# featureform/embeddinghub

Hardware: NVIDIA H100
Metric: k-NN queries/s (higher is better)
Workload: dtype f32

## Files before the change

embeddinghub_b200/csrc/search.cu:

```cuda
#include <cstdio>

#include "kernels.h"

namespace ehb {

cudaError_t launch_search(const WalkPlan& p, const GraphView& g, const float* queries, uint32_t nq, uint32_t k,
                          uint32_t ef, const ResultSink& sink, uint32_t* out_counts, uint32_t* stats, cudaStream_t s) {
  if (nq == 0) return cudaSuccess;
  if (p.bf16 && (!g.vecs16 || !sink.keys)) return cudaErrorInvalidValue;
  return with_dpad(g.dpad, [&](auto d) {
    constexpr uint32_t D = decltype(d)::value;
    return p.bf16 ? SearchShape<D, __nv_bfloat16>::launch(p, g, queries, nq, k, ef, sink, out_counts, stats, s)
                  : SearchShape<D, float>::launch(p, g, queries, nq, k, ef, sink, out_counts, stats, s);
  });
}

cudaError_t beam_warps(const WalkPlan& p, const GraphView& g, int sms, uint64_t nq, uint32_t* warps) {
  return with_dpad(g.dpad, [&](auto d) {
    constexpr uint32_t D = decltype(d)::value;
    return p.bf16 ? BeamShape<D, __nv_bfloat16>::warps(p, sms, nq, warps) : BeamShape<D, float>::warps(p, sms, nq, warps);
  });
}

cudaError_t resident_warps(const void* kern, uint32_t smem, int sms, uint32_t* out) {
  cudaError_t e = cudaFuncSetAttribute(kern, cudaFuncAttributeMaxDynamicSharedMemorySize, (int)smem);
  int per_sm = 0;
  if (e == cudaSuccess) e = cudaOccupancyMaxActiveBlocksPerMultiprocessor(&per_sm, kern, 32, smem);
  if (e != cudaSuccess) return e;
  if (per_sm < 1) return cudaErrorInvalidConfiguration;
  *out = (uint32_t)per_sm * (uint32_t)sms;
  return cudaSuccess;
}

cudaError_t launch_search_beam(const WalkPlan& p, const GraphView& g, const float* queries, uint32_t nq, uint32_t k,
                               uint32_t ef, const ResultSink& sink, uint32_t* out_counts, uint32_t* stats,
                               uint32_t* vtab, uint32_t warps, cudaStream_t s) {
  if (nq == 0) return cudaSuccess;
  if (p.bf16 && (!g.vecs16 || !sink.keys)) return cudaErrorInvalidValue;
  return with_dpad(g.dpad, [&](auto d) {
    constexpr uint32_t D = decltype(d)::value;
    return p.bf16 ? BeamShape<D, __nv_bfloat16>::launch(p, g, queries, nq, k, ef, sink, out_counts, stats, vtab, warps, s)
                  : BeamShape<D, float>::launch(p, g, queries, nq, k, ef, sink, out_counts, stats, vtab, warps, s);
  });
}

void walk_kernel_name(const WalkPlan& p, char* out, size_t out_bytes) {
  if (p.form == WalkForm::team)
    std::snprintf(out, out_bytes, "hnsw_search_team_kernel<NQ=%d,KPL=%d,T=%u,U=%u>", p.nq, p.kpl, p.T, p.U);
  else if (p.form == WalkForm::beam)
    std::snprintf(out, out_bytes, "hnsw_search_beam_kernel<LPV=%d,NQ=%d%s%s>", p.lpv, p.nq,
                  p.hasdel ? ",HASDEL=1" : "", p.bf16 ? ",ROW=bf16" : "");
  else
    std::snprintf(out, out_bytes, "%s<LPV=%d,NQ=%d,KPL=%d%s%s>",
                  p.form == WalkForm::dense  ? "hnsw_search_dense_kernel"
                  : p.form == WalkForm::wide ? "hnsw_search_wide_kernel"
                                             : "hnsw_search_kernel",
                  p.lpv, p.nq, p.kpl, p.hasdel ? ",HASDEL=1" : "", p.bf16 ? ",ROW=bf16" : "");
}

__global__ void pad_rows_kernel(const float* __restrict__ in, float* __restrict__ out, uint64_t n, uint32_t dim,
                                uint32_t dpad, int normalize) {
  uint64_t row = (uint64_t)blockIdx.x * (blockDim.x >> 5) + (threadIdx.x >> 5);
  uint32_t lane = threadIdx.x & 31;
  if (row >= n) return;
  const float* src = in + row * dim;
  float* dst = out + row * dpad;
  float inv = 1.0f;
  if (normalize) {
    float acc = 0.f;
    if (lane == 0) {
      for (uint32_t i = 0; i < dim; ++i) acc = fmaf(src[i], src[i], acc);
      inv = 1.0f / (sqrtf(acc) + 1e-30f);
    }
    inv = __shfl_sync(0xffffffffu, inv, 0);
  }
  for (uint32_t i = lane; i < dpad; i += 32) dst[i] = i < dim ? (normalize ? src[i] * inv : src[i]) : 0.f;
}

cudaError_t launch_pad_rows(const float* in, float* out, uint64_t n, uint32_t dim, uint32_t dpad, bool normalize,
                            cudaStream_t s) {
  if (n == 0) return cudaSuccess;
  uint32_t wpb = 8;
  pad_rows_kernel<<<(unsigned)((n + wpb - 1) / wpb), 32 * wpb, 0, s>>>(in, out, n, dim, dpad, normalize ? 1 : 0);
  return cudaGetLastError();
}

cudaError_t launch_normalize(const float* in, uint32_t in_stride, float* out, uint32_t out_stride, uint64_t n,
                             uint32_t dim, cudaStream_t s) {
  (void)in_stride;
  return launch_pad_rows(in, out, n, dim, out_stride, true, s);
}

__global__ void to_i8_rows_kernel(const float* __restrict__ in, uint32_t dpad, int8_t* __restrict__ codes,
                                  float4* __restrict__ terms, uint64_t n) {
  const uint64_t row = (uint64_t)blockIdx.x * (blockDim.x >> 5) + (threadIdx.x >> 5);
  const uint32_t lane = threadIdx.x & 31;
  if (row >= n) return;
  const float* src = in + row * dpad;
  float mx = 0.f;
  bool finite = true;
  for (uint32_t i = 4 * lane; i < dpad; i += 128) {
    const float4 v = *(const float4*)(src + i);
    finite = finite && isfinite(v.x) && isfinite(v.y) && isfinite(v.z) && isfinite(v.w);
    mx = fmaxf(mx, fmaxf(fmaxf(fabsf(v.x), fabsf(v.y)), fmaxf(fabsf(v.z), fabsf(v.w))));
  }
  finite = __all_sync(0xffffffffu, finite);
  mx = __uint_as_float(__reduce_max_sync(0xffffffffu, __float_as_uint(mx)));
  const float s = (float)((double)mx / 127.0);
  const bool bad = !finite || (s != 0.f && s < 0x1p-126f);
  const double sd = s;
  double rinf = 0.0, r2 = 0.0, x2 = 0.0;
  for (uint32_t i = 4 * lane; i < dpad; i += 128) {
    const float4 v = *(const float4*)(src + i);
    const float xv[4] = {v.x, v.y, v.z, v.w};
    uint32_t packed = 0;
#pragma unroll
    for (int j = 0; j < 4; ++j) {
      const double x = xv[j];
      const double c = bad || s == 0.f ? 0.0 : fmin(fmax(rint(x / sd), -127.0), 127.0);
      const double r = x - sd * c;
      rinf = fmax(rinf, fabs(r));
      r2 = fma(r, r, r2);
      x2 = fma(x, x, x2);
      packed |= (uint32_t)(uint8_t)(int8_t)c << (8 * j);
    }
    *(uint32_t*)(codes + row * dpad + i) = packed;
  }
#pragma unroll
  for (int o = 16; o > 0; o >>= 1) {
    rinf = fmax(rinf, __shfl_xor_sync(0xffffffffu, rinf, o));
    r2 += __shfl_xor_sync(0xffffffffu, r2, o);
    x2 += __shfl_xor_sync(0xffffffffu, x2, o);
  }
  if (lane == 0) {
    const double up = 1.0 + 0x1p-30;
    terms[row] = bad ? make_float4(NAN, NAN, NAN, NAN)
                     : make_float4(s, __double2float_ru(rinf), __double2float_ru(sqrt(r2) * up),
                                   __double2float_ru(sqrt(x2) * up));
  }
}

cudaError_t launch_to_i8(const float* in, uint32_t dpad, int8_t* codes, float4* terms, uint64_t n, cudaStream_t s) {
  if (n == 0) return cudaSuccess;
  to_i8_rows_kernel<<<(unsigned)((n + 7) / 8), 256, 0, s>>>(in, dpad, codes, terms, n);
  return cudaGetLastError();
}

__global__ void sum_stats_kernel(const uint32_t* __restrict__ stats, uint32_t nq, unsigned long long* out) {
  unsigned long long a[kStatWords] = {};
  for (uint32_t i = blockIdx.x * blockDim.x + threadIdx.x; i < nq; i += gridDim.x * blockDim.x) {
    const uint4 s = ((const uint4*)stats)[2 * i], t = ((const uint4*)stats)[2 * i + 1];
    a[0] += s.x, a[1] += s.y, a[2] += s.z, a[3] += s.w ? 1 : 0, a[4] += t.x, a[5] += t.y;
  }
#pragma unroll
  for (int j = 0; j < 6; ++j) {
    for (int o = 16; o > 0; o >>= 1) a[j] += __shfl_xor_sync(0xffffffffu, a[j], o);
    if ((threadIdx.x & 31) == 0) atomicAdd(&out[j], a[j]);
  }
}

cudaError_t launch_sum_stats(const uint32_t* stats, uint32_t nq, unsigned long long* out, cudaStream_t s) {
  cudaError_t e = cudaMemsetAsync(out, 0, kStatWords * sizeof(unsigned long long), s);
  if (e != cudaSuccess) return e;
  if (nq) sum_stats_kernel<<<64, 256, 0, s>>>(stats, nq, out);
  return cudaGetLastError();
}

}
```

embeddinghub_b200/csrc/search_impl.cuh:

```cuda
#pragma once
#include "kernels.h"

namespace ehb {

template <int LPV, int NQ, int KPL, bool HASDEL, int UDIV, class RowT>
__device__ __forceinline__ void search_body(const GraphView& g, const WalkCfg& cfg, const float* __restrict__ queries,
                                            uint32_t nq, uint32_t k, uint32_t ef, const ResultSink& sink,
                                            uint32_t* __restrict__ out_counts, uint32_t* __restrict__ stats,
                                            uint32_t warp_smem) {
  extern __shared__ __align__(128) unsigned char smem[];
  const uint32_t w = threadIdx.x >> 5;
  const uint32_t q = blockIdx.x * (blockDim.x >> 5) + w;
  if (q >= nq) return;
  constexpr bool kKeys = !std::is_same<RowT, float>::value;
  constexpr bool kScreen = !kKeys && screen_shape(LPV, NQ);
  WarpCtx c;
  ctx_init(c, smem + (size_t)w * warp_smem, cfg, g.dpad, (uint32_t)sizeof(RowT));
  float4 qr[NQ];
  if constexpr (wide_shape(LPV, NQ))
    load_query_smem<NQ, RowT>(c, queries + (size_t)q * g.dim, g.dim);
  else
    load_query_regs<LPV, NQ, RowT>(qr, queries + (size_t)q * g.dim, g.dim, c.lane);
  WalkCounters wc = {0, 0, 0, 0};
  UList<KPL> ul;
  ul_clear<KPL>(ul, ef, c.lane);
  if (g.n != 0) {
    uint32_t cur = g.entry;
    if (c.lane == 0) c.cand_id[0] = cur;
    __syncwarp();
    eval_candidates<LPV, NQ, UDIV, RowT, kScreen>(c, walk_rows<RowT>(g), qr, 1, g.metric);
    float curdist = c.cand_dist[0];
    __syncwarp();
    wc.evals = 1;
    greedy_descent<LPV, NQ, UDIV, RowT, kScreen>(c, g, qr, cur, curdist, g.max_level, 0, wc);
    beam_search<LPV, NQ, KPL, true, HASDEL, UDIV, RowT, kScreen>(c, g, qr, ul, cur, curdist, 0, ef, kInvalid, wc);
  }
  uint64_t rk[KPL];
#pragma unroll
  for (int s = 0; s < KPL; ++s) rk[s] = kMaxKey;
  uint32_t found = 0;
  for (uint32_t i = 0; i < k; ++i) {
    uint64_t key = ul_extract_min<KPL>(ul, c.lane);
    if (key == kMaxKey) break;
#pragma unroll
    for (int s = 0; s < KPL; ++s)
      if ((i >> 5) == (uint32_t)s && (i & 31u) == c.lane) rk[s] = key;
    found++;
  }
  if constexpr (kKeys) {
#pragma unroll
    for (int s = 0; s < KPL; ++s) {
      const uint32_t idx = (uint32_t)s * 32u + c.lane;
      if ((uint32_t)s * 32u < k && idx < k) sink.keys[(size_t)q * k + idx] = rk[s];
    }
  } else {
#pragma unroll
    for (int s = 0; s < KPL; ++s) {
      const uint32_t idx = (uint32_t)s * 32u + c.lane;
      if ((uint32_t)s * 32u < k && idx < k) {
        const bool ok = rk[s] != kMaxKey;
        const uint64_t lab = ok ? g.labels[key_id(rk[s])] : 0xFFFFFFFFFFFFFFFFull;
        const float dist = ok ? key_dist(rk[s]) : INFINITY;
        sink_store(sink, (size_t)q * k + idx, lab, dist);
      }
    }
    sink_query_done(sink, q, nq, c.lane);
  }
  if (c.lane == 0) {
    if (out_counts) out_counts[q] = found;
    if (stats) {
      ((uint4*)stats)[2 * q] = make_uint4(wc.hops_upper, wc.hops_base, wc.evals, wc.overflow);
      ((uint4*)stats)[2 * q + 1] = make_uint4(wc.screened, wc.survivors, 0u, 0u);
    }
  }
}

template <class RowT>
constexpr int kWalkMinBlocks = std::is_same<RowT, float>::value ? 0 : 1;
template <int LPV, int NQ, int KPL, bool HASDEL, class RowT>
__global__ void __launch_bounds__(128, (kWalkMinBlocks<RowT>))
    hnsw_search_kernel(GraphView g, WalkCfg cfg, const float* __restrict__ queries, uint32_t nq, uint32_t k, uint32_t ef,
                       const __grid_constant__ ResultSink sink, uint32_t* __restrict__ out_counts,
                       uint32_t* __restrict__ stats, uint32_t warp_smem) {
  search_body<LPV, NQ, KPL, HASDEL, 1, RowT>(g, cfg, queries, nq, k, ef, sink, out_counts, stats, warp_smem);
}

template <int NQ, int KPL>
constexpr int kScreenWalkRegs = NQ <= 6 && KPL <= 8 ? 200 : 255;
template <int LPV, int NQ, int KPL, bool HASDEL>
__global__ void __maxnreg__((kScreenWalkRegs<NQ, KPL>))
    hnsw_search_screen_kernel(GraphView g, WalkCfg cfg, const float* __restrict__ queries, uint32_t nq, uint32_t k,
                              uint32_t ef, const __grid_constant__ ResultSink sink, uint32_t* __restrict__ out_counts,
                              uint32_t* __restrict__ stats, uint32_t warp_smem) {
  search_body<LPV, NQ, KPL, HASDEL, 1, float>(g, cfg, queries, nq, k, ef, sink, out_counts, stats, warp_smem);
}

template <int LPV, int NQ, int KPL, class RowT>
__global__ void __launch_bounds__(128, 5) hnsw_search_dense_kernel(GraphView g, WalkCfg cfg,
                                                                   const float* __restrict__ queries, uint32_t nq,
                                                                   uint32_t k, uint32_t ef,
                                                                   const __grid_constant__ ResultSink sink,
                                                                   uint32_t* __restrict__ out_counts,
                                                                   uint32_t* __restrict__ stats, uint32_t warp_smem) {
  search_body<LPV, NQ, KPL, false, 2, RowT>(g, cfg, queries, nq, k, ef, sink, out_counts, stats, warp_smem);
}

template <int NQ, int KPL, bool HASDEL, class RowT>
__global__ void __launch_bounds__(128, (kWalkMinBlocks<RowT>))
    hnsw_search_wide_kernel(GraphView g, WalkCfg cfg, const float* __restrict__ queries, uint32_t nq, uint32_t k,
                            uint32_t ef, const __grid_constant__ ResultSink sink, uint32_t* __restrict__ out_counts,
                            uint32_t* __restrict__ stats, uint32_t warp_smem) {
  search_body<32, NQ, KPL, HASDEL, 1, RowT>(g, cfg, queries, nq, k, ef, sink, out_counts, stats, warp_smem);
}

using WalkKernel = void (*)(GraphView, WalkCfg, const float*, uint32_t, uint32_t, uint32_t, const ResultSink,
                           uint32_t*, uint32_t*, uint32_t);
template <int LPV, int NQ, int KPL, class RowT>
WalkKernel walk_kernel(const WalkPlan& p) {
  constexpr bool kBf16 = !std::is_same<RowT, float>::value;
  if constexpr (wide_shape(LPV, NQ)) {
    if (p.form != WalkForm::wide) return nullptr;
    return p.hasdel ? hnsw_search_wide_kernel<NQ, KPL, true, RowT> : hnsw_search_wide_kernel<NQ, KPL, false, RowT>;
  } else {
    if (p.form == WalkForm::wide) return nullptr;
    if (p.form == WalkForm::dense) {
      if constexpr (dense_form(kBf16, LPV, NQ, KPL, false))
        if (!p.hasdel) return hnsw_search_dense_kernel<LPV, NQ, KPL, RowT>;
      return nullptr;
    }
    if constexpr (std::is_same<RowT, float>::value && screen_shape(LPV, NQ))
      return p.hasdel ? hnsw_search_screen_kernel<LPV, NQ, KPL, true> : hnsw_search_screen_kernel<LPV, NQ, KPL, false>;
    else
      return p.hasdel ? hnsw_search_kernel<LPV, NQ, KPL, true, RowT> : hnsw_search_kernel<LPV, NQ, KPL, false, RowT>;
  }
}

template <int LPV, int NQ, int KPL, class RowT>
cudaError_t launch_search_t(const WalkPlan& p, const GraphView& g, const float* queries, uint32_t nq, uint32_t k,
                            uint32_t ef, const ResultSink& sink, uint32_t* out_counts, uint32_t* stats,
                            cudaStream_t s) {
  const uint32_t wpb = p.wpb;
  uint32_t wsm = warp_smem_bytes(p.cfg, g.dpad, (uint32_t)sizeof(RowT));
  size_t smem = (size_t)wsm * wpb;
  dim3 grid((nq + wpb - 1) / wpb), block(32 * wpb);
  const WalkKernel kern = walk_kernel<LPV, NQ, KPL, RowT>(p);
  if (!kern) return cudaErrorInvalidValue;
  cudaError_t e = cudaFuncSetAttribute(kern, cudaFuncAttributeMaxDynamicSharedMemorySize, (int)smem);
  if (e != cudaSuccess) return e;
  kern<<<grid, block, smem, s>>>(g, p.cfg, queries, nq, k, ef, sink, out_counts, stats, wsm);
  return cudaGetLastError();
}

template <uint32_t DPAD, class RowT>
cudaError_t SearchShape<DPAD, RowT>::launch(const WalkPlan& p, const GraphView& g, const float* queries, uint32_t nq,
                                            uint32_t k, uint32_t ef, const ResultSink& sink, uint32_t* out_counts,
                                            uint32_t* stats, cudaStream_t s) {
  constexpr int LPV = row_lpv(DPAD * sizeof(RowT)), NQ = row_nq(DPAD, DPAD * sizeof(RowT));
  if (p.lpv != LPV || p.nq != NQ || p.form == WalkForm::team) return cudaErrorInvalidValue;
  switch (p.kpl) {
    case 2: return launch_search_t<LPV, NQ, 2, RowT>(p, g, queries, nq, k, ef, sink, out_counts, stats, s);
    case 4: return launch_search_t<LPV, NQ, 4, RowT>(p, g, queries, nq, k, ef, sink, out_counts, stats, s);
    case 8: return launch_search_t<LPV, NQ, 8, RowT>(p, g, queries, nq, k, ef, sink, out_counts, stats, s);
    case 16: return launch_search_t<LPV, NQ, 16, RowT>(p, g, queries, nq, k, ef, sink, out_counts, stats, s);
    default: return cudaErrorInvalidValue;
  }
}

}
```

embeddinghub_b200/csrc/walk.cuh:

```cuda
#pragma once
#include <cuda_bf16.h>

#include <type_traits>

#include "common.cuh"

namespace ehb {

struct GraphView {
  const float* vecs;
  const uint32_t* links0;
  const uint32_t* up_off;
  const uint32_t* links_up;
  const uint64_t* labels;
  const uint8_t* deleted;
  uint32_t n, dim, dpad, M, M0, entry;
  int32_t max_level;
  int32_t metric;
  const __nv_bfloat16* vecs16;
  const int8_t* codes8;
  const float4* terms8;
};

struct WalkCfg {
// ... 180 lines not shown
  constexpr int V = LaneChunks<RowT, NQ>::V;
  uint32_t sub = lane % LPV;
#pragma unroll
  for (int t = 0; t < NQ; ++t) {
    uint32_t e = (sub + LPV * (t / V)) * 4u * V + 4u * (t % V);
    float4 v;
    v.x = e + 0 < dim ? src[e + 0] : 0.f;
    v.y = e + 1 < dim ? src[e + 1] : 0.f;
    v.z = e + 2 < dim ? src[e + 2] : 0.f;
    v.w = e + 3 < dim ? src[e + 3] : 0.f;
    qr[t] = v;
  }
}
template <int LPV, int NQ, class RowT, class C = LaneChunks<RowT, NQ>>
__device__ __forceinline__ void load_vec_regs(typename C::T (&r)[C::N], const RowT* __restrict__ row,
                                              uint32_t lane) {
  const typename C::T* p = (const typename C::T*)row + (lane % LPV);
#pragma unroll
  for (int t = 0; t < C::N; ++t) r[t] = p[LPV * t];
}

template <int NQ>
__device__ __forceinline__ float partial_dist(const float4 (&v)[NQ], const float4 (&qr)[NQ], int metric) {
  float a0 = 0.f, a1 = 0.f, a2 = 0.f, a3 = 0.f;
  if (metric == 0) {
#pragma unroll
    for (int t = 0; t < NQ; ++t) {
      float dx = qr[t].x - v[t].x, dy = qr[t].y - v[t].y, dz = qr[t].z - v[t].z, dw = qr[t].w - v[t].w;
      a0 = fmaf(dx, dx, a0);
      a1 = fmaf(dy, dy, a1);
      a2 = fmaf(dz, dz, a2);
      a3 = fmaf(dw, dw, a3);
    }
  } else {
#pragma unroll
    for (int t = 0; t < NQ; ++t) {
      a0 = fmaf(qr[t].x, v[t].x, a0);
      a1 = fmaf(qr[t].y, v[t].y, a1);
      a2 = fmaf(qr[t].z, v[t].z, a2);
      a3 = fmaf(qr[t].w, v[t].w, a3);
    }
  }
  return (a0 + a1) + (a2 + a3);
}
template <int LPV>
__device__ __forceinline__ float group_reduce(float acc) {
#pragma unroll
  for (int o = LPV / 2; o > 0; o >>= 1) acc += __shfl_xor_sync(0xffffffffu, acc, o);
  return acc;
}

template <int NQ, class RowT, class C = LaneChunks<RowT, NQ>>
__device__ __forceinline__ float chunk_dist(const typename C::T (&v)[C::N], const float4 (&qr)[NQ], int metric) {
  float4 x[NQ];
#pragma unroll
  for (int j = 0; j < C::N; ++j) widen(v[j], x + j * C::V);
  return partial_dist<NQ>(x, qr, metric);
}
template <class RowT>
__device__ __forceinline__ const RowT* walk_rows(const GraphView& g) {
  if constexpr (std::is_same<RowT, float>::value)
    return g.vecs;
  else
    return g.vecs16;
}

__host__ __device__ constexpr int eval_u(int N, int UDIV) {
  return ((N <= 2 ? 8 : (N <= 4 ? 4 : 2)) / UDIV) > 0 ? (N <= 2 ? 8 : (N <= 4 ? 4 : 2)) / UDIV : 1;
}
template <int NQ, int U = eval_u(NQ, 1), class RowT = float>
__device__ __forceinline__ void eval_direct(WarpCtx& c, const RowT* __restrict__ rows, const float4 (&qr)[NQ],
                                            uint32_t m, int metric) {
  using C = LaneChunks<RowT, NQ>;
  const uint32_t sub = c.lane & 7u, grp = c.lane >> 3;
  __syncwarp();
#pragma unroll 1
  for (uint32_t j0 = 0; j0 < m; j0 += 4 * U) {
    typename C::T v[U][C::N];
#pragma unroll
    for (int u = 0; u < U; ++u) {
      if (j0 + 4u * u < m) {
        uint32_t j = min(j0 + 4u * u + grp, m - 1u);
        const typename C::T* p = (const typename C::T*)(rows + (size_t)c.cand_id[j] * c.dpad) + sub;
#pragma unroll
        for (int t = 0; t < C::N; ++t) v[u][t] = ld_chunk(p + 8 * t);
      }
    }
#pragma unroll
    for (int u = 0; u < U; ++u) {
      if (j0 + 4u * u < m) {
        uint32_t j = j0 + 4u * u + grp;
        float acc = group_reduce<8>(chunk_dist<NQ, RowT>(v[u], qr, metric));
        if (sub == 0 && j < m) c.cand_dist[j] = metric == 0 ? acc : 1.0f - acc;
      }
    }
  }
  __syncwarp();
}

template <class RowT>
__device__ __forceinline__ void issue_rows(WarpCtx& c, const RowT* __restrict__ vecs, uint32_t r, uint32_t m,
                                           uint32_t G, uint32_t vbytes) {
  uint32_t buf = r % c.NG;
  uint32_t first = r * G;
  uint32_t cnt = min(G, m - first);
  if (c.lane == 0) mbar_arrive_expect_tx(&c.mbar[buf], cnt * vbytes);
  __syncwarp();
  if (c.lane < cnt) {
    uint32_t id = c.cand_id[first + c.lane];
    bulk_g2s((RowT*)c.stage + (size_t)(buf * G + c.lane) * c.dpad, vecs + (size_t)id * c.dpad, vbytes, &c.mbar[buf]);
  }
}
template <class RowT>
__device__ __forceinline__ void issue_group(WarpCtx& c, const RowT* __restrict__ vecs, uint32_t r, uint32_t m) {
  issue_rows(c, vecs, r, m, c.G, c.vbytes);
}
template <int NQ, class RowT>
__device__ __forceinline__ void eval_staged(WarpCtx& c, const RowT* __restrict__ vecs, const float4 (&qr)[NQ],
                                            uint32_t m, int metric) {
  const uint32_t rounds = (m + c.G - 1) / c.G;
  const uint32_t pre = min(rounds, c.NG);
  for (uint32_t r = 0; r < pre; ++r) issue_group(c, vecs, r, m);
#pragma unroll 1
  for (uint32_t r = 0; r < rounds; ++r) {
    uint32_t buf = r % c.NG;
    mbar_wait(&c.mbar[buf], (c.phases >> buf) & 1u);
    c.phases ^= (1u << buf);
    uint32_t first = r * c.G;
    uint32_t cnt = min(c.G, m - first);
#pragma unroll 1
    for (uint32_t v0 = 0; v0 < cnt; v0 += 4) {
      float acc[4];
#pragma unroll
      for (int i = 0; i < 4; ++i) {
        uint32_t v = min(v0 + (uint32_t)i, cnt - 1u);
        typename LaneChunks<RowT, NQ>::T x[LaneChunks<RowT, NQ>::N];
        load_vec_regs<32, NQ>(x, (const RowT*)c.stage + (size_t)(buf * c.G + v) * c.dpad, c.lane);
        acc[i] = chunk_dist<NQ, RowT>(x, qr, metric);
      }
#pragma unroll
      for (int o = 16; o > 0; o >>= 1) {
#pragma unroll
        for (int i = 0; i < 4; ++i) acc[i] += __shfl_xor_sync(0xffffffffu, acc[i], o);
      }
      if (c.lane < 4 && v0 + c.lane < cnt) {
        float a = c.lane == 0 ? acc[0] : (c.lane == 1 ? acc[1] : (c.lane == 2 ? acc[2] : acc[3]));
        c.cand_dist[first + v0 + c.lane] = metric == 0 ? a : 1.0f - a;
      }
    }
    __syncwarp();
    if (r + c.NG < rounds) {
      fence_proxy_async();
      issue_group(c, vecs, r + c.NG, m);
    }
  }
  __syncwarp();
}

template <int NQ>
__device__ __forceinline__ void eval_regs(WarpCtx& c, const float* __restrict__ vecs, const float4 (&qr)[NQ],
                                          uint32_t m, int metric) {
  constexpr int SB = NQ <= 24 ? 24 / NQ : 1;
#pragma unroll 1
  for (uint32_t v0 = 0; v0 < m; v0 += SB) {
    float4 x[SB][NQ];
#pragma unroll
    for (int i = 0; i < SB; ++i) {
      const uint32_t v = min(v0 + (uint32_t)i, m - 1u);
      const float4* p = (const float4*)(vecs + (size_t)c.cand_id[v] * c.dpad) + c.lane;
#pragma unroll
      for (int t = 0; t < NQ; ++t) x[i][t] = ld_nc_f4(p + 32 * t);
    }
    float acc[SB];
#pragma unroll
    for (int i = 0; i < SB; ++i) acc[i] = chunk_dist<NQ, float>(x[i], qr, metric);
#pragma unroll
    for (int o = 16; o > 0; o >>= 1) {
#pragma unroll
      for (int i = 0; i < SB; ++i) acc[i] += __shfl_xor_sync(0xffffffffu, acc[i], o);
    }
    if (c.lane < (uint32_t)SB && v0 + c.lane < m) {
      float a = acc[0];
#pragma unroll
      for (int i = 1; i < SB; ++i)
        if (c.lane == (uint32_t)i) a = acc[i];
      c.cand_dist[v0 + c.lane] = metric == 0 ? a : 1.0f - a;
    }
  }
  __syncwarp();
}

template <int NQ, class RowT>
__device__ __forceinline__ void load_query_smem(WarpCtx& c, const float* __restrict__ src, uint32_t dim) {
  constexpr int V = LaneChunks<RowT, NQ>::V;
  float4* qs = (float4*)c.stage + c.lane;
  __syncwarp();
#pragma unroll 4
  for (int t = 0; t < NQ; ++t) {
    const uint32_t e = (c.lane + 32u * (t / V)) * 4u * V + 4u * (t % V);
    float4 v;
    v.x = e + 0 < dim ? src[e + 0] : 0.f;
    v.y = e + 1 < dim ? src[e + 1] : 0.f;
    v.z = e + 2 < dim ? src[e + 2] : 0.f;
    v.w = e + 3 < dim ? src[e + 3] : 0.f;
    qs[32 * t] = v;
  }
  __syncwarp();
}
constexpr int kWideRows = 4;
template <int NQ, class RowT>
__device__ __forceinline__ void eval_wide(WarpCtx& c, const RowT* __restrict__ vecs, uint32_t m, int metric) {
  using C = LaneChunks<RowT, NQ>;
  constexpr int V = C::V, SB = kWideRows, NS = 8 / V;
  static_assert(C::N % NS == 0, "the d-slices tile the row");
  const float4* qs = (const float4*)c.stage + c.lane;
#pragma unroll 1
  for (uint32_t v0 = 0; v0 < m; v0 += SB) {
    const typename C::T* p[SB];
#pragma unroll
    for (int i = 0; i < SB; ++i)
      p[i] = (const typename C::T*)(vecs + (size_t)c.cand_id[min(v0 + (uint32_t)i, m - 1u)] * c.dpad) + c.lane;
    float a[SB][4];
#pragma unroll
    for (int i = 0; i < SB; ++i) a[i][0] = a[i][1] = a[i][2] = a[i][3] = 0.f;
#pragma unroll 1
    for (int j0 = 0; j0 < C::N; j0 += NS) {
      typename C::T x[SB][NS];
#pragma unroll
      for (int i = 0; i < SB; ++i)
#pragma unroll
        for (int j = 0; j < NS; ++j) x[i][j] = ld_chunk(p[i] + 32 * (j0 + j));
#pragma unroll
      for (int j = 0; j < NS; ++j) {
        float4 q[V];
#pragma unroll
        for (int v = 0; v < V; ++v) q[v] = qs[32 * ((j0 + j) * V + v)];
#pragma unroll
        for (int i = 0; i < SB; ++i) {
          float4 r[V];
          widen(x[i][j], r);
#pragma unroll
          for (int v = 0; v < V; ++v) {
            if (metric == 0) {
              const float dx = q[v].x - r[v].x, dy = q[v].y - r[v].y, dz = q[v].z - r[v].z, dw = q[v].w - r[v].w;
              a[i][0] = fmaf(dx, dx, a[i][0]);
              a[i][1] = fmaf(dy, dy, a[i][1]);
              a[i][2] = fmaf(dz, dz, a[i][2]);
              a[i][3] = fmaf(dw, dw, a[i][3]);
            } else {
              a[i][0] = fmaf(q[v].x, r[v].x, a[i][0]);
              a[i][1] = fmaf(q[v].y, r[v].y, a[i][1]);
              a[i][2] = fmaf(q[v].z, r[v].z, a[i][2]);
              a[i][3] = fmaf(q[v].w, r[v].w, a[i][3]);
            }
          }
        }
      }
    }
    float acc[SB];
#pragma unroll
    for (int i = 0; i < SB; ++i) acc[i] = (a[i][0] + a[i][1]) + (a[i][2] + a[i][3]);
#pragma unroll
    for (int o = 16; o > 0; o >>= 1) {
#pragma unroll
      for (int i = 0; i < SB; ++i) acc[i] += __shfl_xor_sync(0xffffffffu, acc[i], o);
    }
    if (c.lane < (uint32_t)SB && v0 + c.lane < m) {
      float d = acc[0];
#pragma unroll
      for (int i = 1; i < SB; ++i)
        if (c.lane == (uint32_t)i) d = acc[i];
      c.cand_dist[v0 + c.lane] = metric == 0 ? d : 1.0f - d;
    }
  }
  __syncwarp();
}

template <int LPV, int NQ, int UDIV = 1, class RowT = float, bool SCREEN = false>
__device__ __forceinline__ void eval_candidates(WarpCtx& c, const RowT* __restrict__ vecs, const float4 (&qr)[NQ],
                                                uint32_t m, int metric) {
  if constexpr (wide_shape(LPV, NQ)) {
    eval_wide<NQ, RowT>(c, vecs, m, metric);
    return;
  }
  if (LPV == 8) {
    eval_direct<NQ, eval_u(LaneChunks<RowT, NQ>::N, UDIV)>(c, vecs, qr, m, metric);
  } else {
    if constexpr (SCREEN) {
      if (!c.staged) {
        eval_regs<NQ>(c, vecs, qr, m, metric);
        return;
      }
    }
    eval_staged<NQ>(c, vecs, qr, m, metric);
  }
}

constexpr int kQMax = 8191;
struct ScreenQuery {
  float l1, l2, a, en, sq;
};
__device__ __forceinline__ ScreenQuery* screen_query(const WarpCtx& c) { return (ScreenQuery*)(c.mbar + 8); }
template <int NQ>
__device__ __forceinline__ uint32_t screen_regs(WarpCtx& c, const GraphView& g, const uint32_t (&qh)[NQ],
                                                const uint32_t (&ql)[NQ], uint32_t m, uint32_t worst_hi,
                                                uint32_t& unsure) {
  constexpr int RB = 96 / NQ;
  const bool in = c.lane < m;
  const uint32_t id = in ? c.cand_id[c.lane] : kInvalid;
  float4 tm = make_float4(0.f, 0.f, 0.f, 0.f);
  if (in) tm = ld_nc_f4(g.terms8 + id);
  int K = 0;
#pragma unroll 1
  for (uint32_t v0 = 0; v0 < m; v0 += RB) {
    uint32_t x[RB][NQ];
#pragma unroll
    for (int i = 0; i < RB; ++i) {
      const uint32_t* p = (const uint32_t*)(g.codes8 + (size_t)c.cand_id[min(v0 + (uint32_t)i, m - 1u)] * c.dpad) +
                          c.lane;
#pragma unroll
      for (int t = 0; t < NQ; ++t) x[i][t] = ld_nc_u32(p + 32 * t);
    }
#pragma unroll
    for (int i = 0; i < RB; ++i) {
      int h = 0, l = 0;
#pragma unroll
      for (int t = 0; t < NQ; ++t) {
        h = __dp4a((int)x[i][t], (int)qh[t], h);
        l = __dp4a((int)x[i][t], (int)ql[t], l);
      }
      const int kv = __reduce_add_sync(0xffffffffu, 128 * h + l);
      if (c.lane == v0 + (uint32_t)i) K = kv;
    }
  }
  float L = 0.f;
  if (in) {
    const ScreenQuery sq = *screen_query(c);
    const float e = (float)c.dpad * 0x1p-24f;
    const float gam = __fdiv_ru(e, 1.0f - e);
    const float se = __fmul_ru(__fmul_ru(tm.x, __int2float_ru(K)), sq.sq);
    float mg = __fmul_ru(__fmul_ru(gam, sq.l2), tm.w);
    mg = __fadd_ru(mg, fminf(__fmul_ru(sq.l1, tm.y), __fmul_ru(sq.l2, tm.z)));
    mg = __fadd_ru(mg, __fmaf_ru(sq.en, __fadd_ru(tm.w, tm.z), sq.a));
    L = __fsub_rd(__fsub_rd(1.0f, se), mg);
  }
  const bool keep = in && !(isfinite(L) && f2ord(L) >= worst_hi);
  const uint32_t mask = __ballot_sync(0xffffffffu, keep);
  const uint32_t pos = __popc(mask & lanemask_lt());
  __syncwarp();
  if (keep) c.cand_id[pos] = id;
  if (unsure) unsure = __reduce_or_sync(0xffffffffu, (keep && ((unsure >> c.lane) & 1u)) ? (1u << pos) : 0u);
  __syncwarp();
  return __popc(mask);
}

template <int KPL>
struct UList {
  uint32_t hi[KPL];
  uint32_t id[KPL];
};
template <int KPL>
__device__ __forceinline__ void ul_clear(UList<KPL>& u, uint32_t ef, uint32_t lane) {
#pragma unroll
  for (int s = 0; s < KPL; ++s) {
    u.hi[s] = ((uint32_t)s * 32u + lane) < ef ? 0xFFFFFFFFu : 0u;
    u.id[s] = kInvalid;
  }
}
template <int KPL>
__device__ __forceinline__ uint32_t ul_worst(const UList<KPL>& u) {
  uint32_t m = u.hi[0];
#pragma unroll
  for (int s = 1; s < KPL; ++s) m = max(m, u.hi[s]);
  return __reduce_max_sync(0xffffffffu, m);
}
template <int KPL>
__device__ __forceinline__ void ul_insert(UList<KPL>& u, uint32_t hi, uint32_t id, uint32_t ef, uint32_t& cnt,
                                          uint32_t& worst_hi, uint32_t lane) {
  bool done = false;
  if (cnt < ef) {
#pragma unroll
    for (int s = 0; s < KPL; ++s) {
      if (!done) {
        uint32_t b = __ballot_sync(0xffffffffu, u.id[s] == kInvalid && u.hi[s] == 0xFFFFFFFFu);
        if (b) {
          if ((int)lane == __ffs(b) - 1) u.hi[s] = hi, u.id[s] = id;
          done = true;
        }
      }
    }
    cnt++;
    if (cnt == ef) worst_hi = ul_worst<KPL>(u);
  } else {
#pragma unroll
    for (int s = 0; s < KPL; ++s) {
      if (!done) {
        uint32_t b = __ballot_sync(0xffffffffu, u.hi[s] == worst_hi && u.id[s] != kInvalid);
        if (b) {
          if ((int)lane == __ffs(b) - 1) u.hi[s] = hi, u.id[s] = id;
          done = true;
        }
      }
    }
    worst_hi = ul_worst<KPL>(u);
  }
}
template <int KPL>
__device__ __forceinline__ uint32_t ul_min_unexpanded(UList<KPL>& u, bool mark, uint32_t lane) {
  uint32_t m = 0xFFFFFFFFu;
#pragma unroll
  for (int s = 0; s < KPL; ++s)
    if (!(u.id[s] & kExpandedFlag)) m = min(m, u.hi[s]);
  m = __reduce_min_sync(0xffffffffu, m);
  uint32_t node = kInvalid;
  bool done = false;
#pragma unroll
  for (int s = 0; s < KPL; ++s) {
    if (!done) {
      uint32_t b = __ballot_sync(0xffffffffu, !(u.id[s] & kExpandedFlag) && u.hi[s] == m);
      if (b) {
        int l = __ffs(b) - 1;
        node = __shfl_sync(0xffffffffu, u.id[s], l);
        if (mark && (int)lane == l) u.id[s] |= kExpandedFlag;
        done = true;
      }
    }
  }
  return node;
}
template <int KPL>
__device__ __forceinline__ uint32_t ul_min_unexpanded_hi(const UList<KPL>& u) {
  uint32_t m = 0xFFFFFFFFu;
#pragma unroll
  for (int s = 0; s < KPL; ++s)
    if (!(u.id[s] & kExpandedFlag)) m = min(m, u.hi[s]);
  return __reduce_min_sync(0xffffffffu, m);
}
template <int KPL>
__device__ __forceinline__ bool ul_contains(const UList<KPL>& u, uint32_t id) {
  bool hit = false;
#pragma unroll
  for (int s = 0; s < KPL; ++s) hit |= u.id[s] != kInvalid && (u.id[s] & kIdMask) == id;
  return __any_sync(0xffffffffu, hit);
}
template <int KPL>
__device__ __forceinline__ uint64_t ul_extract_min(UList<KPL>& u, uint32_t lane) {
  uint32_t m = 0xFFFFFFFFu;
#pragma unroll
  for (int s = 0; s < KPL; ++s)
    if (u.id[s] != kInvalid) m = min(m, u.hi[s]);
  m = __reduce_min_sync(0xffffffffu, m);
  uint64_t out = kMaxKey;
  bool done = false;
#pragma unroll
  for (int s = 0; s < KPL; ++s) {
    if (!done) {
      uint32_t b = __ballot_sync(0xffffffffu, u.id[s] != kInvalid && u.hi[s] == m);
      if (b) {
        int l = __ffs(b) - 1;
        uint32_t id = __shfl_sync(0xffffffffu, u.id[s], l);
        out = ((uint64_t)m << 32) | (id & kIdMask);
        if ((int)lane == l) u.id[s] = kInvalid, u.hi[s] = 0xFFFFFFFFu;
        done = true;
      }
    }
  }
  return out;
}
template <int KPL>
__device__ __forceinline__ void ul_extract_all(WarpCtx& c, UList<KPL>& u) {
  c.cnt = 0;
  for (;;) {
    uint64_t key = ul_extract_min<KPL>(u, c.lane);
    if (key == kMaxKey) break;
    if (c.lane == 0) c.keys[c.cnt] = key;
    c.cnt++;
  }
  __syncwarp();
}

struct SList {
  uint32_t* hi;
  uint32_t* id;
  uint32_t C;
  uint32_t whi, wrow;
  uint32_t uhi, urow;
};
__device__ __forceinline__ void sl_init(SList& u, const WarpCtx& c) {
  u.hi = (uint32_t*)c.keys;
  u.id = u.hi + c.lcap;
  u.C = c.lcap / 32u;
}
__device__ __forceinline__ void sl_scan(SList& u, uint32_t col, bool worst, uint32_t lane) {
  __syncwarp();
  const uint32_t* hc = u.hi + col * u.C;
  const uint32_t* ic = u.id + col * u.C;
  uint32_t wh = 0, wr = kInvalid, uh = 0xFFFFFFFFu, ur = kInvalid;
  for (uint32_t r = lane; r < u.C; r += 32) {
    const uint32_t h = hc[r], d = ic[r];
    if (d != kInvalid && (wr == kInvalid || h > wh)) wh = h, wr = r;
    if (!(d & kExpandedFlag) && (ur == kInvalid || h < uh)) uh = h, ur = r;
  }
  const uint32_t um = __reduce_min_sync(0xffffffffu, ur != kInvalid ? uh : 0xFFFFFFFFu);
  const uint32_t ub = __ballot_sync(0xffffffffu, ur != kInvalid && uh == um);
  const uint32_t urow = ub ? __shfl_sync(0xffffffffu, ur, __ffs(ub) - 1) : kInvalid;
  if (lane == col) u.uhi = um, u.urow = urow;
  if (worst) {
    const uint32_t wm = __reduce_max_sync(0xffffffffu, wr != kInvalid ? wh : 0u);
    const uint32_t wb = __ballot_sync(0xffffffffu, wr != kInvalid && wh == wm);
    const uint32_t wrow = wb ? __shfl_sync(0xffffffffu, wr, __ffs(wb) - 1) : kInvalid;
    if (lane == col) u.whi = wm, u.wrow = wrow;
  }
}
__device__ __forceinline__ void ul_clear(SList& u, uint32_t ef, uint32_t lane) {
  (void)ef;
  __syncwarp();
  for (uint32_t i = lane; i < 32u * u.C; i += 32) u.hi[i] = 0, u.id[i] = kInvalid;
  u.whi = 0, u.wrow = kInvalid, u.uhi = 0xFFFFFFFFu, u.urow = kInvalid;
  __syncwarp();
}
__device__ __forceinline__ void ul_insert(SList& u, uint32_t hi, uint32_t id, uint32_t ef, uint32_t& cnt,
                                          uint32_t& worst_hi, uint32_t lane) {
  if (cnt < ef) {
    const uint32_t col = cnt & 31u, row = cnt >> 5;
    if (lane == col) {
      u.hi[col * u.C + row] = hi, u.id[col * u.C + row] = id;
      if (u.wrow == kInvalid || hi > u.whi) u.whi = hi, u.wrow = row;
      if (u.urow == kInvalid || hi < u.uhi) u.uhi = hi, u.urow = row;
    }
    __syncwarp();
    cnt++;
    if (cnt == ef) worst_hi = __reduce_max_sync(0xffffffffu, u.wrow != kInvalid ? u.whi : 0u);
  } else {
    const uint32_t b = __ballot_sync(0xffffffffu, u.wrow != kInvalid && u.whi == worst_hi);
    const uint32_t col = __ffs(b) - 1;
    const uint32_t row = __shfl_sync(0xffffffffu, u.wrow, col);
    if (lane == col) u.hi[col * u.C + row] = hi, u.id[col * u.C + row] = id;
    sl_scan(u, col, true, lane);
    worst_hi = __reduce_max_sync(0xffffffffu, u.wrow != kInvalid ? u.whi : 0u);
  }
}
__device__ __forceinline__ uint64_t sl_take_min(SList& u, bool mark, uint32_t lane) {
  const uint32_t m = __reduce_min_sync(0xffffffffu, u.urow != kInvalid ? u.uhi : 0xFFFFFFFFu);
  const uint32_t b = __ballot_sync(0xffffffffu, u.urow != kInvalid && u.uhi == m);
  if (!b) return kMaxKey;
  const uint32_t col = __ffs(b) - 1;
  const uint32_t at = col * u.C + __shfl_sync(0xffffffffu, u.urow, col);
  const uint32_t node = u.id[at];
  if (mark) {
    __syncwarp();
    if (lane == col) u.id[at] = node | kExpandedFlag;
    sl_scan(u, col, false, lane);
  }
  return ((uint64_t)m << 32) | node;
}
__device__ __forceinline__ uint32_t ul_min_unexpanded(SList& u, bool mark, uint32_t lane) {
  const uint64_t key = sl_take_min(u, mark, lane);
  return key == kMaxKey ? kInvalid : (uint32_t)key;
}
__device__ __forceinline__ uint32_t ul_min_unexpanded_hi(const SList& u) {
  return __reduce_min_sync(0xffffffffu, u.urow != kInvalid ? u.uhi : 0xFFFFFFFFu);
}
__device__ __forceinline__ bool ul_contains(const SList& u, uint32_t id) {
  bool hit = false;
  for (uint32_t i = (uint32_t)threadIdx.x & 31u; i < 32u * u.C; i += 32) hit |= u.id[i] != kInvalid && (u.id[i] & kIdMask) == id;
  return __any_sync(0xffffffffu, hit);
}
__device__ __forceinline__ void sl_begin_extract(SList& u, uint32_t lane) {
  __syncwarp();
  for (uint32_t i = lane; i < 32u * u.C; i += 32)
    if (u.id[i] != kInvalid) u.id[i] &= kIdMask;
  for (uint32_t col = 0; col < 32; ++col) sl_scan(u, col, false, lane);
}

__device__ __forceinline__ uint32_t list_insert(WarpCtx& c, uint64_t key, uint32_t limit) {
  const uint32_t id = key_id(key);
  uint32_t pos = 0;
  uint32_t dup = 0;
  for (uint32_t base = 0; base < c.cnt; base += 32) {
    uint32_t i = base + c.lane;
    uint64_t k = i < c.cnt ? c.keys[i] : kMaxKey;
    pos += __popc(__ballot_sync(0xffffffffu, k < key));
    dup |= __ballot_sync(0xffffffffu, i < c.cnt && key_id(k) == id);
  }
  if (dup || pos >= limit) return kInvalid;
  const uint32_t newcnt = min(c.cnt + 1u, limit);
  for (int base = (int)((newcnt - 1u) & ~31u); base >= (int)(pos & ~31u); base -= 32) {
    uint32_t i = (uint32_t)base + c.lane;
    bool in = i >= pos && i < newcnt;
    uint64_t v = key;
    if (in && i > pos) v = c.keys[i - 1];
    __syncwarp();
    if (in) c.keys[i] = v;
  }
  __syncwarp();
  c.cnt = newcnt;
  return pos;
}

struct WalkCounters {
  uint32_t hops_upper, hops_base, evals, overflow, screened, survivors;
};

__device__ __forceinline__ uint32_t load_row(const GraphView& g, uint32_t node, int level, uint32_t lane) {
  const uint32_t* row;
  uint32_t width;
  if (level == 0) {
    row = g.links0 + (size_t)node * g.M0;
    width = g.M0;
  } else {
    row = g.links_up + (size_t)(g.up_off[node] + (uint32_t)(level - 1)) * g.M;
    width = g.M;
  }
  uint32_t v = row[min(lane, width - 1u)];
  return lane < width ? v : kInvalid;
}

template <int LPV, int NQ, int UDIV = 1, class RowT = float, bool SCREEN = false>
__device__ __forceinline__ void greedy_descent(WarpCtx& c, const GraphView& g, const float4 (&qr)[NQ], uint32_t& cur,
                                               float& curdist, int from_level, int to_level_excl,
                                               WalkCounters& wc) {
  for (int level = from_level; level > to_level_excl; --level) {
    bool changed = true;
    while (changed) {
      changed = false;
      __syncwarp();
      uint32_t nb = load_row(g, cur, level, c.lane);
      uint32_t mask = __ballot_sync(0xffffffffu, nb != kInvalid);
      uint32_t m = __popc(mask);
      wc.hops_upper++;
      if (!m) break;
      if (nb != kInvalid) c.cand_id[__popc(mask & lanemask_lt())] = nb;
      __syncwarp();
      wc.evals += m;
      eval_candidates<LPV, NQ, UDIV, RowT, SCREEN>(c, walk_rows<RowT>(g), qr, m, g.metric);
      float bd = c.lane < m ? c.cand_dist[c.lane] : INFINITY;
      uint32_t bl = c.lane;
#pragma unroll
      for (int o = 16; o > 0; o >>= 1) {
        float od = __shfl_xor_sync(0xffffffffu, bd, o);
        uint32_t ol = __shfl_xor_sync(0xffffffffu, bl, o);
        if (od < bd || (od == bd && ol < bl)) bd = od, bl = ol;
      }
      if (bd < curdist) {
        curdist = bd;
        cur = c.cand_id[bl];
        changed = true;
      }
      __syncwarp();
    }
  }
}

__device__ __forceinline__ void dq_push(WarpCtx& c, uint32_t& dn, uint32_t hi, uint32_t id, uint32_t bound,
                                        uint32_t& overflow) {
  if (dn < c.dcap) {
    if (c.lane == 0) c.dq_hi[dn] = hi, c.dq_id[dn] = id;
    dn++;
  } else {
    uint32_t w = 0, wp = 0;
    for (uint32_t i = c.lane; i < dn; i += 32)
      if (c.dq_hi[i] >= w) w = c.dq_hi[i], wp = i;
    uint32_t wm = __reduce_max_sync(0xffffffffu, w);
    uint32_t b = __ballot_sync(0xffffffffu, w == wm);
    uint32_t pos = __shfl_sync(0xffffffffu, wp, __ffs(b) - 1);
    if (hi < wm && c.lane == 0) c.dq_hi[pos] = hi, c.dq_id[pos] = id;
    if (max(hi, wm) <= bound) overflow = 1;
  }
  __syncwarp();
}
__device__ __forceinline__ uint32_t dq_min(const WarpCtx& c, uint32_t dn, uint32_t& hi_out) {
  uint32_t m = 0xFFFFFFFFu, mp = kInvalid;
  for (uint32_t i = c.lane; i < dn; i += 32)
    if (c.dq_hi[i] < m) m = c.dq_hi[i], mp = i;
  uint32_t mm = __reduce_min_sync(0xffffffffu, m);
  uint32_t b = __ballot_sync(0xffffffffu, m == mm && mp != kInvalid);
  hi_out = mm;
  return b ? __shfl_sync(0xffffffffu, mp, __ffs(b) - 1) : kInvalid;
}

template <int LPV, int NQ, int KPL, bool PREFETCH, bool HASDEL, int UDIV = 1, class RowT = float, bool SCREEN = false,
          class Set = UList<KPL>>
__device__ __forceinline__ void beam_search(WarpCtx& c, const GraphView& g, const float4 (&qr)[NQ], Set& u,
                                            uint32_t ep, float epdist, int level, uint32_t ef, uint32_t exclude,
                                            WalkCounters& wc) {
  static_assert(!SCREEN || (screen_shape(LPV, NQ) && std::is_same<RowT, float>::value), "no screen for this shape");
  const bool screen = SCREEN && g.codes8 && g.metric == 1;
  uint32_t qh[NQ], ql[NQ];
  if (screen) {
    float mx = 0.f, l1 = 0.f, l2 = 0.f;
#pragma unroll
    for (int t = 0; t < NQ; ++t) {
      const float v[4] = {qr[t].x, qr[t].y, qr[t].z, qr[t].w};
#pragma unroll
      for (int j = 0; j < 4; ++j) {
        mx = fmaxf(mx, fabsf(v[j]));
        l1 = __fadd_ru(l1, fabsf(v[j]));
        l2 = __fmaf_ru(v[j], v[j], l2);
      }
    }
#pragma unroll
    for (int o = 16; o > 0; o >>= 1) {
      l1 = __fadd_ru(l1, __shfl_xor_sync(0xffffffffu, l1, o));
      l2 = __fadd_ru(l2, __shfl_xor_sync(0xffffffffu, l2, o));
    }
    mx = __uint_as_float(__reduce_max_sync(0xffffffffu, __float_as_uint(mx)));
    float sq = mx / (float)kQMax;
    if (!(sq >= 0x1p-126f && sq <= 0x1.fffffep127f)) sq = 0.f;
    double e2 = 0.0;
#pragma unroll
    for (int t = 0; t < NQ; ++t) {
      const float v[4] = {qr[t].x, qr[t].y, qr[t].z, qr[t].w};
      uint32_t h = 0, l = 0;
#pragma unroll
      for (int j = 0; j < 4; ++j) {
        const int k = sq != 0.f ? max(-kQMax, min(kQMax, __float2int_rn(v[j] / sq))) : 0;
        const double e = (double)v[j] - (double)sq * (double)k;
        e2 = __fma_ru(e, e, e2);
        const int kh = (k + 64) >> 7;
        h |= (uint32_t)(kh & 0xFF) << (8 * j);
        l |= (uint32_t)((k - 128 * kh) & 0xFF) << (8 * j);
      }
      qh[t] = h;
      ql[t] = l;
    }
#pragma unroll
    for (int o = 16; o > 0; o >>= 1) e2 = __dadd_ru(e2, __shfl_xor_sync(0xffffffffu, e2, o));
    if (c.lane == 0)
      *screen_query(c) = {l1, __fsqrt_ru(l2), __fmul_ru((float)g.dpad, __fmaf_ru(mx, 0x1p-125f, 0x1p-124f)),
                          __double2float_ru(__dsqrt_ru(e2)), sq};
    __syncwarp();
  }
  hash_clear(c);
  ul_clear(u, ef, c.lane);
  const uint8_t* __restrict__ del = (HASDEL && c.dcap) ? g.deleted : nullptr;
  uint32_t dn = 0;
  uint32_t ovf = 0;
  if (c.lane == 0) {
    hash_insert(c, ep, ovf);
    if (exclude != kInvalid) hash_insert(c, exclude, ovf);
  }
  __syncwarp();
  uint32_t cnt = 0;
  uint32_t worst_hi = 0xFFFFFFFFu;
  bool ovf_any = false;
  const bool ep_result = ep != exclude && !(del && del[ep]);
  if (ep_result) ul_insert(u, f2ord(epdist), ep, ef, cnt, worst_hi, c.lane);
  uint32_t node = ep;
  if (ep_result) node = ul_min_unexpanded(u, true, c.lane);
  uint32_t nb = load_row(g, node, level, c.lane);
  for (;;) {
    if (level == 0) wc.hops_base++; else wc.hops_upper++;
    if (HASDEL && wc.hops_base + wc.hops_upper > 64u * ef + 65536u) break;
    __syncwarp();
    const uint32_t spec = ul_min_unexpanded(u, false, c.lane);
    uint32_t spec_row = kInvalid;
    if (spec != kInvalid) spec_row = load_row(g, spec & kIdMask, level, c.lane);
    bool is_new = false;
    uint32_t o = 0;
    if (nb != kInvalid && nb != exclude) is_new = hash_insert(c, nb, o);
    ovf |= o;
    __syncwarp();
    uint32_t mask = __ballot_sync(0xffffffffu, is_new);
    uint32_t m = __popc(mask);
    if (m) {
      const uint32_t pos = __popc(mask & lanemask_lt());
      if (is_new) c.cand_id[pos] = nb;
      uint32_t unsure = (HASDEL && del) ? __reduce_or_sync(0xffffffffu, (is_new && o) ? (1u << pos) : 0u) : 0u;
      __syncwarp();
      wc.evals += m;
      if (SCREEN && screen && cnt >= ef) {
        wc.screened += m;
        m = screen_regs<NQ>(c, g, qh, ql, m, worst_hi, unsure);
        wc.survivors += m;
        eval_regs<NQ>(c, g.vecs, qr, m, 1);
      } else {
        eval_candidates<LPV, NQ, UDIV, RowT, SCREEN>(c, walk_rows<RowT>(g), qr, m, g.metric);
      }
      if (PREFETCH && LPV == 8 && c.prefetch && spec_row != kInvalid) {
        const char* pv = (const char*)(walk_rows<RowT>(g) + (size_t)spec_row * g.dpad);
#pragma unroll
        for (int b = 0; b < NQ * 8 * 16 * (int)sizeof(RowT) / 4; b += 128) prefetch_l2(pv + b);
      }
      uint32_t myhi = 0xFFFFFFFFu, myid = kInvalid;
      if (c.lane < m) myhi = f2ord(c.cand_dist[c.lane]), myid = c.cand_id[c.lane];
      const bool mydel = HASDEL && del && c.lane < m && del[myid];
      __syncwarp();
      ovf_any = ovf_any || __any_sync(0xffffffffu, ovf);
      uint32_t qual = __ballot_sync(0xffffffffu, c.lane < m && (cnt < ef || myhi < worst_hi));
      const uint32_t delmask = (HASDEL && del) ? __ballot_sync(0xffffffffu, mydel) : 0u;
      while (qual) {
        int j = __ffs(qual) - 1;
        qual &= qual - 1;
        uint32_t hj = __shfl_sync(0xffffffffu, myhi, j);
        uint32_t ij = __shfl_sync(0xffffffffu, myid, j);
        if (cnt >= ef && hj >= worst_hi) continue;
        if (HASDEL && ((delmask >> j) & 1u)) {
          if (!((unsure >> j) & 1u)) dq_push(c, dn, hj, ij, cnt >= ef ? worst_hi : 0xFFFFFFFFu, ovf);
          continue;
        }
        if (ovf_any && ul_contains(u, ij)) continue;
        ul_insert(u, hj, ij, ef, cnt, worst_hi, c.lane);
        if (PREFETCH && c.lane == 0) prefetch_l2(g.links0 + (size_t)ij * g.M0);
      }
    }
    if (HASDEL && dn) {
      uint32_t dhi;
      const uint32_t dpos = dq_min(c, dn, dhi);
      if (dhi < ul_min_unexpanded_hi(u)) {
        if (cnt >= ef && dhi > worst_hi) break;
        node = c.dq_id[dpos];
        __syncwarp();
        if (c.lane == 0) c.dq_hi[dpos] = c.dq_hi[dn - 1], c.dq_id[dpos] = c.dq_id[dn - 1];
        dn--;
        __syncwarp();
        nb = load_row(g, node, level, c.lane);
        continue;
      }
    }
    node = ul_min_unexpanded(u, true, c.lane);
    if (node == kInvalid) break;
    nb = (node == spec) ? spec_row : load_row(g, node, level, c.lane);
  }
  wc.overflow |= (ovf_any || __any_sync(0xffffffffu, ovf)) ? 1u : 0u;
}

}
```

Before: 520,700.

## Apply int8 screening during greedy descent and prefetch only improving links

Result: faster. 538,100 (median of 6 runs) (+3.3%).

```diff
diff --git a/embeddinghub_b200/csrc/search.cu b/embeddinghub_b200/csrc/search.cu
--- a/embeddinghub_b200/csrc/search.cu
+++ b/embeddinghub_b200/csrc/search.cu
@@ -150,10 +150,10 @@
   unsigned long long a[kStatWords] = {};
   for (uint32_t i = blockIdx.x * blockDim.x + threadIdx.x; i < nq; i += gridDim.x * blockDim.x) {
     const uint4 s = ((const uint4*)stats)[2 * i], t = ((const uint4*)stats)[2 * i + 1];
-    a[0] += s.x, a[1] += s.y, a[2] += s.z, a[3] += s.w ? 1 : 0, a[4] += t.x, a[5] += t.y;
+    a[0] += s.x, a[1] += s.y, a[2] += s.z, a[3] += s.w ? 1 : 0, a[4] += t.x, a[5] += t.y, a[6] += t.z;
   }
 #pragma unroll
-  for (int j = 0; j < 6; ++j) {
+  for (int j = 0; j < 7; ++j) {
     for (int o = 16; o > 0; o >>= 1) a[j] += __shfl_xor_sync(0xffffffffu, a[j], o);
     if ((threadIdx.x & 31) == 0) atomicAdd(&out[j], a[j]);
   }
diff --git a/embeddinghub_b200/csrc/search_impl.cuh b/embeddinghub_b200/csrc/search_impl.cuh
--- a/embeddinghub_b200/csrc/search_impl.cuh
+++ b/embeddinghub_b200/csrc/search_impl.cuh
@@ -25,6 +25,9 @@
   UList<KPL> ul;
   ul_clear<KPL>(ul, ef, c.lane);
   if (g.n != 0) {
+    QueryPlanes<NQ> qp;
+    if constexpr (kScreen)
+      if (walk_screens(g)) screen_setup<NQ>(c, g, qr, qp);
     uint32_t cur = g.entry;
     if (c.lane == 0) c.cand_id[0] = cur;
     __syncwarp();
@@ -32,8 +35,8 @@
     float curdist = c.cand_dist[0];
     __syncwarp();
     wc.evals = 1;
-    greedy_descent<LPV, NQ, UDIV, RowT, kScreen>(c, g, qr, cur, curdist, g.max_level, 0, wc);
-    beam_search<LPV, NQ, KPL, true, HASDEL, UDIV, RowT, kScreen>(c, g, qr, ul, cur, curdist, 0, ef, kInvalid, wc);
+    greedy_descent<LPV, NQ, UDIV, RowT, kScreen>(c, g, qr, cur, curdist, g.max_level, 0, wc, &qp);
+    beam_search<LPV, NQ, KPL, true, HASDEL, UDIV, RowT, kScreen>(c, g, qr, ul, cur, curdist, 0, ef, kInvalid, wc, &qp);
   }
   uint64_t rk[KPL];
 #pragma unroll
@@ -70,7 +73,7 @@
     if (out_counts) out_counts[q] = found;
     if (stats) {
       ((uint4*)stats)[2 * q] = make_uint4(wc.hops_upper, wc.hops_base, wc.evals, wc.overflow);
-      ((uint4*)stats)[2 * q + 1] = make_uint4(wc.screened, wc.survivors, 0u, 0u);
+      ((uint4*)stats)[2 * q + 1] = make_uint4(wc.screened, wc.survivors, wc.screened_upper, 0u);
     }
   }
 }
diff --git a/embeddinghub_b200/csrc/walk.cuh b/embeddinghub_b200/csrc/walk.cuh
--- a/embeddinghub_b200/csrc/walk.cuh
+++ b/embeddinghub_b200/csrc/walk.cuh
@@ -506,9 +506,59 @@
 };
 __device__ __forceinline__ ScreenQuery* screen_query(const WarpCtx& c) { return (ScreenQuery*)(c.mbar + 8); }
 template <int NQ>
-__device__ __forceinline__ uint32_t screen_regs(WarpCtx& c, const GraphView& g, const uint32_t (&qh)[NQ],
-                                                const uint32_t (&ql)[NQ], uint32_t m, uint32_t worst_hi,
-                                                uint32_t& unsure) {
+struct QueryPlanes {
+  uint32_t h[NQ], l[NQ];
+};
+__device__ __forceinline__ bool walk_screens(const GraphView& g) { return g.codes8 && g.metric == 1; }
+template <int NQ>
+__device__ __forceinline__ void screen_setup(WarpCtx& c, const GraphView& g, const float4 (&qr)[NQ],
+                                             QueryPlanes<NQ>& qp) {
+  float mx = 0.f, l1 = 0.f, l2 = 0.f;
+#pragma unroll
+  for (int t = 0; t < NQ; ++t) {
+    const float v[4] = {qr[t].x, qr[t].y, qr[t].z, qr[t].w};
+#pragma unroll
+    for (int j = 0; j < 4; ++j) {
+      mx = fmaxf(mx, fabsf(v[j]));
+      l1 = __fadd_ru(l1, fabsf(v[j]));
+      l2 = __fmaf_ru(v[j], v[j], l2);
+    }
+  }
+#pragma unroll
+  for (int o = 16; o > 0; o >>= 1) {
+    l1 = __fadd_ru(l1, __shfl_xor_sync(0xffffffffu, l1, o));
+    l2 = __fadd_ru(l2, __shfl_xor_sync(0xffffffffu, l2, o));
+  }
+  mx = __uint_as_float(__reduce_max_sync(0xffffffffu, __float_as_uint(mx)));
+  float sq = mx / (float)kQMax;
+  if (!(sq >= 0x1p-126f && sq <= 0x1.fffffep127f)) sq = 0.f;
+  double e2 = 0.0;
+#pragma unroll
+  for (int t = 0; t < NQ; ++t) {
+    const float v[4] = {qr[t].x, qr[t].y, qr[t].z, qr[t].w};
+    uint32_t h = 0, l = 0;
+#pragma unroll
+    for (int j = 0; j < 4; ++j) {
+      const int k = sq != 0.f ? max(-kQMax, min(kQMax, __float2int_rn(v[j] / sq))) : 0;
+      const double e = (double)v[j] - (double)sq * (double)k;
+      e2 = __fma_ru(e, e, e2);
+      const int kh = (k + 64) >> 7;
+      h |= (uint32_t)(kh & 0xFF) << (8 * j);
+      l |= (uint32_t)((k - 128 * kh) & 0xFF) << (8 * j);
+    }
+    qp.h[t] = h;
+    qp.l[t] = l;
+  }
+#pragma unroll
+  for (int o = 16; o > 0; o >>= 1) e2 = __dadd_ru(e2, __shfl_xor_sync(0xffffffffu, e2, o));
+  if (c.lane == 0)
+    *screen_query(c) = {l1, __fsqrt_ru(l2), __fmul_ru((float)g.dpad, __fmaf_ru(mx, 0x1p-125f, 0x1p-124f)),
+                        __double2float_ru(__dsqrt_ru(e2)), sq};
+  __syncwarp();
+}
+template <int NQ>
+__device__ __forceinline__ uint32_t screen_regs(WarpCtx& c, const GraphView& g, const QueryPlanes<NQ>& qp, uint32_t m,
+                                                uint32_t worst_hi, uint32_t& unsure) {
   constexpr int RB = 96 / NQ;
   const bool in = c.lane < m;
   const uint32_t id = in ? c.cand_id[c.lane] : kInvalid;
@@ -530,8 +580,8 @@
       int h = 0, l = 0;
 #pragma unroll
       for (int t = 0; t < NQ; ++t) {
-        h = __dp4a((int)x[i][t], (int)qh[t], h);
-        l = __dp4a((int)x[i][t], (int)ql[t], l);
+        h = __dp4a((int)x[i][t], (int)qp.h[t], h);
+        l = __dp4a((int)x[i][t], (int)qp.l[t], l);
       }
       const int kv = __reduce_add_sync(0xffffffffu, 128 * h + l);
       if (c.lane == v0 + (uint32_t)i) K = kv;
@@ -803,7 +853,7 @@
 }
 
 struct WalkCounters {
-  uint32_t hops_upper, hops_base, evals, overflow, screened, survivors;
+  uint32_t hops_upper, hops_base, evals, overflow, screened, survivors, screened_upper;
 };
 
 __device__ __forceinline__ uint32_t load_row(const GraphView& g, uint32_t node, int level, uint32_t lane) {
@@ -823,7 +873,8 @@
 template <int LPV, int NQ, int UDIV = 1, class RowT = float, bool SCREEN = false>
 __device__ __forceinline__ void greedy_descent(WarpCtx& c, const GraphView& g, const float4 (&qr)[NQ], uint32_t& cur,
                                                float& curdist, int from_level, int to_level_excl,
-                                               WalkCounters& wc) {
+                                               WalkCounters& wc, const QueryPlanes<NQ>* qp = nullptr) {
+  const bool screen = SCREEN && walk_screens(g);
   for (int level = from_level; level > to_level_excl; --level) {
     bool changed = true;
     while (changed) {
@@ -837,7 +888,16 @@
       if (nb != kInvalid) c.cand_id[__popc(mask & lanemask_lt())] = nb;
       __syncwarp();
       wc.evals += m;
-      eval_candidates<LPV, NQ, UDIV, RowT, SCREEN>(c, walk_rows<RowT>(g), qr, m, g.metric);
+      if (SCREEN && screen) {
+        uint32_t unsure = 0;
+        wc.screened += m;
+        wc.screened_upper += m;
+        m = screen_regs<NQ>(c, g, *qp, m, f2ord(curdist), unsure);
+        wc.survivors += m;
+        eval_regs<NQ>(c, g.vecs, qr, m, 1);
+      } else {
+        eval_candidates<LPV, NQ, UDIV, RowT, SCREEN>(c, walk_rows<RowT>(g), qr, m, g.metric);
+      }
       float bd = c.lane < m ? c.cand_dist[c.lane] : INFINITY;
       uint32_t bl = c.lane;
 #pragma unroll
@@ -887,54 +947,9 @@
           class Set = UList<KPL>>
 __device__ __forceinline__ void beam_search(WarpCtx& c, const GraphView& g, const float4 (&qr)[NQ], Set& u,
                                             uint32_t ep, float epdist, int level, uint32_t ef, uint32_t exclude,
-                                            WalkCounters& wc) {
+                                            WalkCounters& wc, const QueryPlanes<NQ>* qp = nullptr) {
   static_assert(!SCREEN || (screen_shape(LPV, NQ) && std::is_same<RowT, float>::value), "no screen for this shape");
-  const bool screen = SCREEN && g.codes8 && g.metric == 1;
-  uint32_t qh[NQ], ql[NQ];
-  if (screen) {
-    float mx = 0.f, l1 = 0.f, l2 = 0.f;
-#pragma unroll
-    for (int t = 0; t < NQ; ++t) {
-      const float v[4] = {qr[t].x, qr[t].y, qr[t].z, qr[t].w};
-#pragma unroll
-      for (int j = 0; j < 4; ++j) {
-        mx = fmaxf(mx, fabsf(v[j]));
-        l1 = __fadd_ru(l1, fabsf(v[j]));
-        l2 = __fmaf_ru(v[j], v[j], l2);
-      }
-    }
-#pragma unroll
-    for (int o = 16; o > 0; o >>= 1) {
-      l1 = __fadd_ru(l1, __shfl_xor_sync(0xffffffffu, l1, o));
-      l2 = __fadd_ru(l2, __shfl_xor_sync(0xffffffffu, l2, o));
-    }
-    mx = __uint_as_float(__reduce_max_sync(0xffffffffu, __float_as_uint(mx)));
-    float sq = mx / (float)kQMax;
-    if (!(sq >= 0x1p-126f && sq <= 0x1.fffffep127f)) sq = 0.f;
-    double e2 = 0.0;
-#pragma unroll
-    for (int t = 0; t < NQ; ++t) {
-      const float v[4] = {qr[t].x, qr[t].y, qr[t].z, qr[t].w};
-      uint32_t h = 0, l = 0;
-#pragma unroll
-      for (int j = 0; j < 4; ++j) {
-        const int k = sq != 0.f ? max(-kQMax, min(kQMax, __float2int_rn(v[j] / sq))) : 0;
-        const double e = (double)v[j] - (double)sq * (double)k;
-        e2 = __fma_ru(e, e, e2);
-        const int kh = (k + 64) >> 7;
-        h |= (uint32_t)(kh & 0xFF) << (8 * j);
-        l |= (uint32_t)((k - 128 * kh) & 0xFF) << (8 * j);
-      }
-      qh[t] = h;
-      ql[t] = l;
-    }
-#pragma unroll
-    for (int o = 16; o > 0; o >>= 1) e2 = __dadd_ru(e2, __shfl_xor_sync(0xffffffffu, e2, o));
-    if (c.lane == 0)
-      *screen_query(c) = {l1, __fsqrt_ru(l2), __fmul_ru((float)g.dpad, __fmaf_ru(mx, 0x1p-125f, 0x1p-124f)),
-                          __double2float_ru(__dsqrt_ru(e2)), sq};
-    __syncwarp();
-  }
+  const bool screen = SCREEN && walk_screens(g);
   hash_clear(c);
   ul_clear(u, ef, c.lane);
   const uint8_t* __restrict__ del = (HASDEL && c.dcap) ? g.deleted : nullptr;
@@ -975,7 +990,7 @@
       wc.evals += m;
       if (SCREEN && screen && cnt >= ef) {
         wc.screened += m;
-        m = screen_regs<NQ>(c, g, qh, ql, m, worst_hi, unsure);
+        m = screen_regs<NQ>(c, g, *qp, m, worst_hi, unsure);
         wc.survivors += m;
         eval_regs<NQ>(c, g.vecs, qr, m, 1);
       } else {
@@ -993,6 +1008,7 @@
       ovf_any = ovf_any || __any_sync(0xffffffffu, ovf);
       uint32_t qual = __ballot_sync(0xffffffffu, c.lane < m && (cnt < ef || myhi < worst_hi));
       const uint32_t delmask = (HASDEL && del) ? __ballot_sync(0xffffffffu, mydel) : 0u;
+      uint32_t next_hi = (SCREEN && screen) ? ul_min_unexpanded_hi(u) : 0xFFFFFFFFu;
       while (qual) {
         int j = __ffs(qual) - 1;
         qual &= qual - 1;
@@ -1005,7 +1021,10 @@
         }
         if (ovf_any && ul_contains(u, ij)) continue;
         ul_insert(u, hj, ij, ef, cnt, worst_hi, c.lane);
-        if (PREFETCH && c.lane == 0) prefetch_l2(g.links0 + (size_t)ij * g.M0);
+        if (PREFETCH && (!(SCREEN && screen) || hj < next_hi)) {
+          next_hi = hj;
+          if (c.lane == 0) prefetch_l2(g.links0 + (size_t)ij * g.M0);
+        }
       }
     }
     if (HASDEL && dn) {
```
